# HyHuang1995/sp_orb_slam

Measured on AMD Instinct MI355X. Metric: frames/sec SuperPoint extract (752x480, 1k kpts), higher is better.
Workload: dtype f32

## Files before the change

sp_orb_slam_amd/csrc/conv_f32.hip:

```cpp
#include <type_traits>
#include <utility>

#include "spfe_kernels.h"
#include "../../include/spfe_exact_math.h"

namespace spfe {

typedef float f32x16 __attribute__((ext_vector_type(16)));

template <int KS, int TH>
struct Geo {
  static constexpr int HALO = KS / 2;
  static constexpr int ROWS = TH + 2 * HALO;
  static constexpr int COLS = 32 + 2 * HALO;
  static constexpr int ROWP = (KS == 3) ? 36 : 32;
  static constexpr int PLANE_RAW = ROWS * ROWP;
  static constexpr int PLANE = PLANE_RAW + ((2 - PLANE_RAW % 8) + 8) % 8;
};

typedef int i32x4 __attribute__((ext_vector_type(4)));
#define SPFE_OOB 0x80000000u

template <int NITER, int NWITER>
struct Pipe {
// ... 19 lines not shown
};

template <int MT, int NT, bool POOL, bool RELU, int E>
__device__ __forceinline__ void epi_store(const EpiCtx<NT> &e, const f32x16 (&acc)[MT][NT]) {
  constexpr int NEPI_ = POOL ? (MT / 2) * NT * 8 : MT * NT * 16;
  if constexpr (E >= NEPI_) {
    return;
  } else if constexpr (!POOL) {
    constexpr int j = E / (MT * 16), i = (E / 16) % MT, r = E % 16;
    constexpr int xr = (r & 3) + 8 * (r >> 2);
    float v = acc[i][j][r] + e.bias[j];
    if (RELU) v = v > 0.0f ? v : 0.0f;
    const unsigned off = (xr < e.xlim && i < e.ylim) ? e.obase[j] + i * e.rowstep + xr * e.pixstep : SPFE_OOB;
    __builtin_amdgcn_raw_buffer_store_b32(__float_as_int(v), e.rout, off, 0, 0);
  } else {
    constexpr int ip = E / (NT * 8), j = (E / 8) % NT, r = 2 * (E % 8), i0 = 2 * ip;
    constexpr int xr = (r & 3) + 8 * (r >> 2);
    float v00 = acc[i0][j][r] + e.bias[j], v01 = acc[i0][j][r + 1] + e.bias[j];
    float v10 = acc[i0 + 1][j][r] + e.bias[j], v11 = acc[i0 + 1][j][r + 1] + e.bias[j];
    if (RELU) {
      v00 = v00 > 0.0f ? v00 : 0.0f;
      v01 = v01 > 0.0f ? v01 : 0.0f;
      v10 = v10 > 0.0f ? v10 : 0.0f;
      v11 = v11 > 0.0f ? v11 : 0.0f;
    }
    const float m0 = v00 > v01 ? v00 : v01;
    const float m1 = v10 > v11 ? v10 : v11;
    const float v = m0 > m1 ? m0 : m1;
    const unsigned off = (xr < e.xlim && i0 < e.ylim) ? e.obase[j] + ip * e.rowstep + (xr >> 1) * e.pixstep : SPFE_OOB;
    __builtin_amdgcn_raw_buffer_store_b32(__float_as_int(v), e.rout, off, 0, 0);
  }
}

constexpr int F1_PROWS = 12, F1_PCOLS = 36, F1_PATCH = F1_PROWS * F1_PCOLS;

template <int NITER>
struct Fuse1a {
  float4 w[9], bias;
  float px[9];
  float4 o;
  unsigned pb[NITER];
  const float *patch;
  float *patch_next;
  const float *wsrc;
  const float *bsrc;
  __amdgpu_buffer_rsrc_t rimg;
  unsigned poff[2];
  unsigned pidx[2];
  unsigned pval[2];
  bool fill;
};
struct NoFuse {};

constexpr int F1_SUBS = 10;
template <int NITER, int IT, int SUB, int PLANE, int NWITER>
__device__ __forceinline__ void fuse_piece(Fuse1a<NITER> &z, Pipe<NITER, NWITER> &c) {
  if constexpr (SUB == 0) {
    const unsigned b = z.pb[IT] == ~0u ? 0u : z.pb[IT];
#pragma unroll
    for (int t = 0; t < 9; ++t) z.px[t] = z.patch[b + (t / 3) * F1_PCOLS + t % 3];
  } else if constexpr (SUB <= 8) {
    constexpr int j = (SUB - 1) / 2, half = (SUB - 1) % 2;
    float acc = half == 0 ? 0.0f : (j == 0 ? z.o.x : (j == 1 ? z.o.y : (j == 2 ? z.o.z : z.o.w)));
#pragma unroll
    for (int t = half * 5; t < (half == 0 ? 5 : 9); ++t) {
      const float wt = j == 0 ? z.w[t].x : (j == 1 ? z.w[t].y : (j == 2 ? z.w[t].z : z.w[t].w));
      acc = __builtin_fmaf(z.px[t], wt, acc);
    }
    if constexpr (half == 1) {
      const float bj = j == 0 ? z.bias.x : (j == 1 ? z.bias.y : (j == 2 ? z.bias.z : z.bias.w));
      acc = acc + bj;
      acc = acc > 0.0f ? acc : 0.0f;
      if (c.voff[IT] == SPFE_OOB) acc = 0.0f;
    }
    if constexpr (j == 0) z.o.x = acc;
    else if constexpr (j == 1) z.o.y = acc;
    else if constexpr (j == 2) z.o.z = acc;
    else z.o.w = acc;
  } else {
    float *d = c.nA + c.dst[IT];
    d[0] = z.o.x;
    d[PLANE] = z.o.y;
    d[2 * PLANE] = z.o.z;
    d[3 * PLANE] = z.o.w;
  }
}

template <int STEP, int NSTEP, bool FIRST, int KC, int KS, int MT, int NT, int PLANE, int ROWP, int NITER,
          int NWITER, bool POOL, bool RELU, bool FUSE, class FZ>
// ... 2 lines not shown
                                        const EpiCtx<NT> &e, FZ &fz) {
  if constexpr (STEP < NSTEP) {
    constexpr int NLDA = FUSE ? 0 : NITER;
    constexpr int NLD = NLDA + NWITER;
    constexpr int L0 = 1, W0 = NSTEP - NLD - 1;
    constexpr int NEPI = POOL ? (MT / 2) * NT * 8 : MT * NT * 16;
    constexpr int EPS = (NEPI + (NSTEP - 3)) / (NSTEP - 2);
    constexpr int cur = STEP & 1, nxt = cur ^ 1;
    static_assert(L0 + NLD <= W0, "loads and LDS writes of a stage must not overlap");
    constexpr int M = MT * NT;
#pragma unroll
    for (int m = 0; m < M; ++m) {
      if (m == 0) {
        if constexpr (STEP + 1 < NSTEP) {
          constexpr int tap = (STEP + 1) / (KC / 2), t = (STEP + 1) % (KC / 2);
          constexpr int dy = tap / KS, dx = tap % KS;
#pragma unroll
          for (int i = 0; i < MT; ++i) {
            if constexpr (KC / 2 <= 8) a[nxt][i] = c.at[t][(i + dy) * ROWP + dx];
            else a[nxt][i] = c.at[0][(2 * t) * PLANE + (i + dy) * ROWP + dx];
          }
#pragma unroll
          for (int j = 0; j < NT; ++j) bb[nxt][j] = c.bBase[j * (KS * KS * KC * 32) + (tap * KC + 2 * t) * 32];
        }
      }
      if (m == 1 % M) {
        if constexpr (STEP >= L0 && STEP - L0 < NLD) {
          constexpr int it = STEP - L0;
          if constexpr (it < NLDA) {
            const i32x4 v = __builtin_amdgcn_raw_buffer_load_b128(c.rin, c.voff[it], 0, 0);
            c.va[it] = make_float4(__int_as_float(v.x), __int_as_float(v.y), __int_as_float(v.z), __int_as_float(v.w));
          } else {
            constexpr int wi = it - NLDA;
            const i32x4 v = __builtin_amdgcn_raw_buffer_load_b128(c.rw, c.woff[wi], 0, 0);
            c.vw[wi] = make_float4(__int_as_float(v.x), __int_as_float(v.y), __int_as_float(v.z), __int_as_float(v.w));
          }
        }
      }
      if (m == 2 % M) {
        if constexpr (FIRST && STEP >= 1) {
          constexpr int e0 = (STEP - 1) * EPS;
          [&]<int... Qs>(std::integer_sequence<int, Qs...>) {
            (epi_store<MT, NT, POOL, RELU, e0 + Qs>(e, accPrev), ...);
          }(std::make_integer_sequence<int, EPS>{});
        }
      }
      if (m == 3 % M) {
        if constexpr (STEP >= W0 && STEP - W0 < NLD) {
          constexpr int it = STEP - W0;
          if constexpr (it < NLDA) {
            float *d = c.nA + c.dst[it];
            d[0] = c.va[it].x;
            d[PLANE] = c.va[it].y;
            d[2 * PLANE] = c.va[it].z;
            d[3 * PLANE] = c.va[it].w;
          } else {
            constexpr int wi = it - NLDA;
            *reinterpret_cast<float4 *>(reinterpret_cast<char *>(c.nW) + c.woff[wi]) = c.vw[wi];
          }
        }
      }
      if (m == 1 % M) {
        if constexpr (FUSE) {
          constexpr int F0 = 12;
          static_assert(L0 + NLD <= F0 && F0 + F1_SUBS * NITER <= NSTEP, "fused conv1a schedule does not fit the stage");
          if constexpr (STEP >= F0 && STEP < F0 + F1_SUBS * NITER)
            fuse_piece<NITER, (STEP - F0) / F1_SUBS, (STEP - F0) % F1_SUBS, PLANE, NWITER>(fz, c);
        }
      }
      if (m == 3 % M) {
        if constexpr (FUSE) {
          static_assert(58 < W0, "fused conv1a schedule does not fit the stage");
          if constexpr (STEP >= 2 && STEP < 11) fz.w[STEP - 2] = *reinterpret_cast<const float4 *>(fz.wsrc + (STEP - 2) * 64);
          if constexpr (STEP == 11) fz.bias = *reinterpret_cast<const float4 *>(fz.bsrc);
          if constexpr (STEP == 50) {
            if (fz.fill) {
              fz.pval[0] = __builtin_amdgcn_raw_buffer_load_b8(fz.rimg, fz.poff[0], 0, 0);
              fz.pval[1] = __builtin_amdgcn_raw_buffer_load_b8(fz.rimg, fz.poff[1], 0, 0);
            }
          }
          if constexpr (STEP == 58) {
            if (fz.fill) {
              if (fz.pidx[0] < F1_PATCH) fz.patch_next[fz.pidx[0]] = spfe_pixel_to_float((uint8_t)fz.pval[0]);
              if (fz.pidx[1] < F1_PATCH) fz.patch_next[fz.pidx[1]] = spfe_pixel_to_float((uint8_t)fz.pval[1]);
            }
          }
        }
      }
      __builtin_amdgcn_sched_barrier(0);
      {
        const int i = m / NT, j = m % NT;
        if constexpr (FIRST && STEP == 0) {
          f32x16 z;
#pragma unroll
          for (int r = 0; r < 16; ++r) z[r] = 0.0f;
          acc[i][j] = __builtin_amdgcn_mfma_f32_32x32x2f32(a[cur][i], bb[cur][j], z, 0, 0, 0);
        } else {
          acc[i][j] = __builtin_amdgcn_mfma_f32_32x32x2f32(a[cur][i], bb[cur][j], acc[i][j], 0, 0, 0);
        }
      }
      __builtin_amdgcn_sched_barrier(0);
    }
    k_steps<STEP + 1, NSTEP, FIRST, KC, KS, MT, NT, PLANE, ROWP, NITER, NWITER, POOL, RELU, FUSE, FZ>(a, bb, acc, accPrev, c, e, fz);
  }
}

template <int LAYER, int CIN, int KS, int KC, int WM, int WN, int MT, int NT, bool POOL, bool RELU>
__global__ __launch_bounds__(64 * WM * WN, 1) void conv_f32_kernel(ConvParams p) {
  constexpr int TH = WM * MT;
  using G = Geo<KS, TH>;
  constexpr int TAPS = KS * KS;
  constexpr int NCHUNK = CIN / KC;
  constexpr int PLANE = G::PLANE;
  constexpr int ROWP = G::ROWP;
  constexpr int BUF = KC * PLANE + TAPS * KC * 64;
  static_assert(WM * WN == 4 || WM * WN == 8, "4 or 8 waves per workgroup");
  constexpr int NTHR = 64 * WM * WN;
  static_assert(WN * NT == 2, "64 output channels per workgroup");
  static_assert(!POOL || MT % 2 == 0, "pooling needs row pairs per wave");
  static_assert((KC * PLANE) % 4 == 0 && BUF % 4 == 0, "weight slabs must stay 16B aligned");
  constexpr int Q = KC / 4;
  constexpr int NITEM = G::ROWS * G::COLS * Q;
  constexpr int NITER = (NITEM + NTHR - 1) / NTHR;
  constexpr int NW4 = TAPS * KC * 16;
  constexpr int NWITER = (NW4 + NTHR - 1) / NTHR;
  constexpr int NSTEP = TAPS * (KC / 2);
  constexpr int SLAB_BYTES = TAPS * KC * 64 * 4;

  constexpr bool FUSE = LAYER == 2;
  static_assert(!FUSE || (CIN == 64 && KS == 3 && KC == 16 && TH == 8), "fused conv1a is conv1b's first operand");
  using FZ = typename std::conditional<FUSE, Fuse1a<NITER>, NoFuse>::type;

  extern __shared__ __attribute__((aligned(16))) float smem[];

  const int tid = threadIdx.x;
  const int lane = tid & 63;
  const int wave = __builtin_amdgcn_readfirstlane(tid >> 6);
  const int hi = lane >> 5, l31 = lane & 31;
  const int wm = wave % WM, wn = wave / WM;
  const int H = p.H, W = p.W;

  const int total = p.nblk * p.tiles_x * p.tiles_y * p.B;
  const int first = p.item_lo, count = (p.item_hi > 0 ? p.item_hi : total) - first;
  const int xcd = blockIdx.x & 7, gi = blockIdx.x >> 3, gper = gridDim.x >> 3;
  const int lo = first + (int)((long)count * xcd / 8), hi_w = first + (int)((long)count * (xcd + 1) / 8);
  int w = lo + gi;
  if (w >= hi_w) return;

  int i_nb, i_tx, i_ty, i_b;
  {
    int t = w;
    i_nb = t % p.nblk; t /= p.nblk;
    i_tx = t % p.tiles_x; t /= p.tiles_x;
    i_ty = t % p.tiles_y; i_b = t / p.tiles_y;
  }
  int d_nb, d_tx, d_ty, d_b;
  {
    int t = gper;
    d_nb = t % p.nblk; t /= p.nblk;
    d_tx = t % p.tiles_x; t /= p.tiles_x;
    d_ty = t % p.tiles_y; d_b = t / p.tiles_y;
  }

  const unsigned in_pix_bytes = (unsigned)p.in_stride * 4u;
  const unsigned frame_in_bytes = (unsigned)H * W * in_pix_bytes;
  const int Ho = POOL ? H >> 1 : H, Wo = POOL ? W >> 1 : W;
  const unsigned out_pix_bytes = (unsigned)p.out_stride * 4u;
  const unsigned frame_out_bytes = (unsigned)Ho * Wo * out_pix_bytes;

  Pipe<NITER, NWITER> c;
  int prow[NITER], pcol[NITER];
  unsigned pqb[NITER];
#pragma unroll
  for (int it = 0; it < NITER; ++it) {
    const int i = tid + it * NTHR;
    const int qq = i % Q, pix = i / Q;
    prow[it] = i < NITEM ? pix / G::COLS - G::HALO : (1 << 20);
    pcol[it] = pix % G::COLS - G::HALO;
    pqb[it] = qq * 16;
    c.dst[it] = i < NITEM ? (qq * 4) * PLANE + (pix / G::COLS) * ROWP + pix % G::COLS
                          : (ROWP > G::COLS ? (tid % G::ROWS) * ROWP + G::COLS : G::PLANE_RAW);
  }
#pragma unroll
  for (int it = 0; it < NWITER; ++it) c.woff[it] = ((tid + it * NTHR) % NW4) * 16;

  auto aim_tile = [&](int tx, int ty) {
#pragma unroll
    for (int it = 0; it < NITER; ++it) {
      const int gy = ty * TH + prow[it], gx = tx * 32 + pcol[it];
      c.voff[it] = ((unsigned)gy < (unsigned)H && (unsigned)gx < (unsigned)W)
                       ? (unsigned)(gy * W + gx) * in_pix_bytes + pqb[it]
                       : SPFE_OOB;
    }
  };
  auto aim_stage = [&](int nb, int b, int chunk, bool valid) {
    const float *base = p.in + (size_t)b * H * W * p.in_stride + p.in_choff + chunk * KC;
    c.rin = __builtin_amdgcn_make_buffer_rsrc(const_cast<float *>(base), 0, valid ? frame_in_bytes : 0u, 0x00020000);
    const float *wb = p.wpack + ((size_t)nb * NCHUNK + chunk) * (TAPS * KC * 64);
    c.rw = __builtin_amdgcn_make_buffer_rsrc(const_cast<float *>(wb), 0, valid ? (unsigned)SLAB_BYTES : 0u, 0x00020000);
  };

  aim_tile(i_tx, i_ty);
  aim_stage(i_nb, i_b, 0, true);
  FZ fz;
  [[maybe_unused]] float *sP = smem + 2 * BUF;
  [[maybe_unused]] int pcur = 0;
  [[maybe_unused]] int php[2] = {0, 0}, pwp[2] = {0, 0};
  if constexpr (FUSE) {
    const int qq = tid % Q;
#pragma unroll
    for (int it = 0; it < NITER; ++it) {
      const int i = tid + it * 256, pix = i / Q;
      fz.pb[it] = i < NITEM ? (unsigned)((pix / G::COLS) * F1_PCOLS + pix % G::COLS) : ~0u;
    }
#pragma unroll
    for (int k = 0; k < 2; ++k) {
      const int i = tid + k * 256;
      fz.pidx[k] = i < F1_PATCH ? (unsigned)i : 0xffffu;
      php[k] = i / F1_PCOLS;
      pwp[k] = i % F1_PCOLS;
      fz.poff[k] = SPFE_OOB;
      fz.pval[k] = 0u;
    }
    fz.fill = false;
    fz.patch = sP;
    fz.patch_next = sP + F1_PATCH;
    fz.rimg = __builtin_amdgcn_make_buffer_rsrc(const_cast<uint8_t *>(p.img), 0, 0u, 0x00020000);
    fz.wsrc = p.w1a + qq * 4;
    fz.bsrc = p.b1a + qq * 4;
    {
      const uint8_t *ib = p.img + (size_t)i_b * H * W;
#pragma unroll
      for (int k = 0; k < 2; ++k) {
        const int gy = i_ty * TH - 2 + php[k], gx = i_tx * 32 - 2 + pwp[k];
        const bool in = (unsigned)gy < (unsigned)H && (unsigned)gx < (unsigned)W;
        if (fz.pidx[k] < F1_PATCH) sP[fz.pidx[k]] = in ? spfe_pixel_to_float(ib[(size_t)gy * W + gx]) : 0.0f;
      }
    }
    __syncthreads();
#pragma unroll
    for (int t = 0; t < 9; ++t) fz.w[t] = *reinterpret_cast<const float4 *>(fz.wsrc + t * 64);
    fz.bias = *reinterpret_cast<const float4 *>(fz.bsrc);
    c.nA = smem;
    [&]<int... I>(std::integer_sequence<int, I...>) {
      (fuse_piece<NITER, I / F1_SUBS, I % F1_SUBS, PLANE, NWITER>(fz, c), ...);
    }(std::make_integer_sequence<int, F1_SUBS * NITER>{});
  } else {
#pragma unroll
    for (int it = 0; it < NITER; ++it) {
      const i32x4 v = __builtin_amdgcn_raw_buffer_load_b128(c.rin, c.voff[it], 0, 0);
      c.va[it] = make_float4(__int_as_float(v.x), __int_as_float(v.y), __int_as_float(v.z), __int_as_float(v.w));
    }
  }
#pragma unroll
  for (int it = 0; it < NWITER; ++it) {
    const i32x4 v = __builtin_amdgcn_raw_buffer_load_b128(c.rw, c.woff[it], 0, 0);
    c.vw[it] = make_float4(__int_as_float(v.x), __int_as_float(v.y), __int_as_float(v.z), __int_as_float(v.w));
  }
  if constexpr (!FUSE) {
#pragma unroll
    for (int it = 0; it < NITER; ++it) {
      float *d = smem + c.dst[it];
      d[0] = c.va[it].x;
      d[PLANE] = c.va[it].y;
      d[2 * PLANE] = c.va[it].z;
      d[3 * PLANE] = c.va[it].w;
// ... 8 lines not shown
#pragma unroll
  for (int i = 0; i < MT; ++i)
#pragma unroll
    for (int j = 0; j < NT; ++j)
#pragma unroll
      for (int r = 0; r < 16; ++r) { accA[i][j][r] = 0.0f; accB[i][j][r] = 0.0f; }

  int buf = 0;
  EpiCtx<NT> epi;
  epi.rout = __builtin_amdgcn_make_buffer_rsrc(p.out, 0, 0u, 0x00020000);
#pragma unroll
  for (int j = 0; j < NT; ++j) { epi.obase[j] = SPFE_OOB; epi.bias[j] = 0.0f; }
  epi.xlim = 0; epi.ylim = 0; epi.rowstep = 0; epi.pixstep = out_pix_bytes;
  bool more = true;

  auto aim_epi = [&](EpiCtx<NT> &e, int nb, int tx, int ty, int b) {
    float *obase = p.out + (size_t)b * Ho * Wo * p.out_stride + p.out_choff;
    e.rout = __builtin_amdgcn_make_buffer_rsrc(obase, 0, frame_out_bytes, 0x00020000);
    const int y0 = ty * TH + wm * MT, x0 = tx * 32 + 4 * hi;
    e.xlim = W - x0;
    e.ylim = H - y0;
    e.rowstep = (unsigned)Wo * out_pix_bytes;
    e.pixstep = out_pix_bytes;
#pragma unroll
    for (int j = 0; j < NT; ++j) {
      const int co = nb * 64 + (wn * NT + j) * 32 + l31;
      const unsigned pix = POOL ? (unsigned)((y0 >> 1) * Wo + (x0 >> 1)) : (unsigned)(y0 * W + x0);
      e.obase[j] = co < p.cout_real ? pix * out_pix_bytes + (unsigned)co * 4u : SPFE_OOB;
      e.bias[j] = p.bias[co];
    }
  };

  EpiCtx<NT> epi_next;
  auto run_tile = [&](f32x16(&acc)[MT][NT], const f32x16(&accPrev)[MT][NT]) {
    int n_nb = i_nb + d_nb, n_tx = i_tx + d_tx, n_ty = i_ty + d_ty, n_b = i_b + d_b;
    if (n_nb >= p.nblk) { n_nb -= p.nblk; ++n_tx; }
    if (n_tx >= p.tiles_x) { n_tx -= p.tiles_x; ++n_ty; }
    if (n_ty >= p.tiles_y) { n_ty -= p.tiles_y; ++n_b; }
    const bool have_next_item = w + gper < hi_w;
    aim_epi(epi_next, i_nb, i_tx, i_ty, i_b);
#pragma unroll 1
    for (int chunk = 0; chunk < NCHUNK; ++chunk) {
      const bool last = chunk == NCHUNK - 1;
      if (!last) {
        aim_stage(i_nb, i_b, chunk + 1, true);
      } else {
        aim_tile(n_tx, n_ty);
        aim_stage(n_nb, n_b, 0, have_next_item);
      }
      if constexpr (FUSE) {
        const int produced = last ? 0 : chunk + 1;
        const int qq = tid % Q;
        fz.wsrc = p.w1a + produced * KC + qq * 4;
        fz.bsrc = p.b1a + produced * KC + qq * 4;
        fz.patch = sP + (last ? pcur ^ 1 : pcur) * F1_PATCH;
        fz.patch_next = sP + (pcur ^ 1) * F1_PATCH;
        fz.fill = chunk == NCHUNK - 2 && have_next_item;
        if (fz.fill) {
          fz.rimg = __builtin_amdgcn_make_buffer_rsrc(const_cast<uint8_t *>(p.img) + (size_t)n_b * H * W, 0,
                                                      (unsigned)(H * W), 0x00020000);
#pragma unroll
          for (int k = 0; k < 2; ++k) {
            const int gy = n_ty * TH - 2 + php[k], gx = n_tx * 32 - 2 + pwp[k];
            fz.poff[k] = ((unsigned)gy < (unsigned)H && (unsigned)gx < (unsigned)W) ? (unsigned)(gy * W + gx) : SPFE_OOB;
          }
        }
      }
      float *cA = smem + buf * BUF;
      c.nA = smem + (buf ^ 1) * BUF;
      c.nW = c.nA + KC * PLANE;
#pragma unroll
      for (int t = 0; t < (KC / 2 <= 8 ? KC / 2 : 1); ++t)
        c.at[t] = cA + (2 * t + hi) * PLANE + (wm * MT) * ROWP + l31;
      c.bBase = cA + KC * PLANE + (wn * NT) * (TAPS * KC * 32) + hi * 32 + l31;
      float a[2][MT], bb[2][NT];
#pragma unroll
      for (int i = 0; i < MT; ++i) a[0][i] = c.at[0][i * ROWP];
#pragma unroll
      for (int j = 0; j < NT; ++j) bb[0][j] = c.bBase[j * (TAPS * KC * 32)];
      if (chunk == 0)
        k_steps<0, NSTEP, true, KC, KS, MT, NT, PLANE, ROWP, NITER, NWITER, POOL, RELU, FUSE, FZ>(a, bb, acc, accPrev, c, epi, fz);
      else
        k_steps<0, NSTEP, false, KC, KS, MT, NT, PLANE, ROWP, NITER, NWITER, POOL, RELU, FUSE, FZ>(a, bb, acc, accPrev, c, epi, fz);
      __syncthreads();
      buf ^= 1;
    }
    epi = epi_next;
    if constexpr (FUSE) pcur ^= 1;
    more = have_next_item;
    w += gper;
    i_nb = n_nb; i_tx = n_tx; i_ty = n_ty; i_b = n_b;
  };

  bool lastA = true;
  while (true) {
    run_tile(accA, accB);
    lastA = true;
    if (!more) break;
    run_tile(accB, accA);
    lastA = false;
    if (!more) break;
  }
  {
    constexpr int NEPI = POOL ? (MT / 2) * NT * 8 : MT * NT * 16;
    auto flush = [&](const f32x16(&acc)[MT][NT]) {
      [&]<int... E>(std::integer_sequence<int, E...>) {
        (epi_store<MT, NT, POOL, RELU, E>(epi, acc), ...);
      }(std::make_integer_sequence<int, NEPI>{});
    };
    if (lastA) flush(accA); else flush(accB);
  }
}

template <int LAYER, int CIN, int KS, int KC, int WM, int WN, int MT, int NT, bool POOL, bool RELU>
static hipError_t launch_one(const ConvParams &p, hipStream_t s) {
  constexpr int TH = WM * MT;
  using G = Geo<KS, TH>;
  constexpr size_t lds = (2 * (size_t)(KC * G::PLANE + KS * KS * KC * 64) + (LAYER == 2 ? 2 * F1_PATCH : 0)) * sizeof(float);
  static_assert(lds <= 160 * 1024, "double buffer must fit the 160 KB LDS");
  auto k = conv_f32_kernel<LAYER, CIN, KS, KC, WM, WN, MT, NT, POOL, RELU>;
  static bool attr_done[64] = {};
  int dev = 0;
  (void)hipGetDevice(&dev);
  if (dev < 0 || dev >= 64 || !attr_done[dev]) {
    hipError_t e = hipFuncSetAttribute(reinterpret_cast<const void *>(k),
                                       hipFuncAttributeMaxDynamicSharedMemorySize, (int)lds);
    if (e != hipSuccess) return e;
    if (dev >= 0 && dev < 64) attr_done[dev] = true;
  }
  const int total = p.nblk * p.tiles_x * p.tiles_y * p.B;
  int grid = p.num_cus > 0 ? p.num_cus : 256;
  grid &= ~7;
  if (grid < 8) grid = 8;
  (void)total;
  hipLaunchKernelGGL(k, dim3(grid), dim3(64 * WM * WN), lds, s, p);
  return hipGetLastError();
}

int conv_kc(int ksize) { return ksize == 3 ? 16 : 64; }
int conv_tile_rows(int tile_mode) { return tile_mode == 1 ? 4 : (tile_mode == 2 || tile_mode == 4 ? 16 : (tile_mode == 3 ? 2 : 8)); }

hipError_t launch_conv_f32(const ConvParams &p, int cin, int ksize, bool pool, bool relu,
                           int tile_mode, int layer_tag, hipStream_t s) {
  const bool small_tile = tile_mode == 1;
  if (tile_mode == 3 && ksize == 3 && relu && !pool) {
    if (cin == 64) return launch_one<0, 64, 3, 16, 2, 2, 1, 1, false, true>(p, s);
    if (cin == 128) return launch_one<0, 128, 3, 16, 2, 2, 1, 1, false, true>(p, s);
    return hipErrorInvalidValue;
  }
  if (tile_mode == 4 && ksize == 3 && relu && pool && cin == 64 && layer_tag == 1)
    return launch_one<1, 64, 3, 16, 4, 1, 4, 2, true, true>(p, s);
  if (tile_mode == 2 && ksize == 3 && relu) {
    if (layer_tag == 1 && cin == 64 && pool) return launch_one<1, 64, 3, 16, 8, 1, 2, 2, true, true>(p, s);
    if (cin == 64 && pool) return launch_one<0, 64, 3, 16, 8, 1, 2, 2, true, true>(p, s);
    if (cin == 64 && !pool) return launch_one<0, 64, 3, 16, 8, 1, 2, 2, false, true>(p, s);
    if (cin == 128 && pool) return launch_one<0, 128, 3, 16, 8, 1, 2, 2, true, true>(p, s);
    if (cin == 128 && !pool) return launch_one<0, 128, 3, 16, 8, 1, 2, 2, false, true>(p, s);
    return hipErrorInvalidValue;
  }
  if (layer_tag == 1 && cin == 64 && ksize == 3 && pool && relu && !small_tile)
    return launch_one<1, 64, 3, 16, 4, 1, 2, 2, true, true>(p, s);
  if (layer_tag == 2 && cin == 64 && ksize == 3 && pool && relu && !small_tile && p.img && p.w1a && p.b1a)
    return launch_one<2, 64, 3, 16, 4, 1, 2, 2, true, true>(p, s);
#define SPFE_CONV(CIN_, KS_, KC_, WM_, WN_, MT_, NT_, POOL_, RELU_)                       \
  if (cin == CIN_ && ksize == KS_ && pool == POOL_ && relu == RELU_ &&                    \
      small_tile == (WM_ * MT_ == 4))                                                     \
    return launch_one<0, CIN_, KS_, KC_, WM_, WN_, MT_, NT_, POOL_, RELU_>(p, s);
  SPFE_CONV(64, 3, 16, 4, 1, 2, 2, true, true)
  SPFE_CONV(64, 3, 16, 4, 1, 2, 2, false, true)
  SPFE_CONV(128, 3, 16, 4, 1, 2, 2, true, true)
  SPFE_CONV(128, 3, 16, 4, 1, 2, 2, false, true)
  SPFE_CONV(64, 3, 16, 2, 2, 2, 1, true, true)
  SPFE_CONV(64, 3, 16, 2, 2, 2, 1, false, true)
  SPFE_CONV(128, 3, 16, 2, 2, 2, 1, true, true)
  SPFE_CONV(128, 3, 16, 2, 2, 2, 1, false, true)
  SPFE_CONV(256, 1, 64, 2, 2, 2, 1, false, false)
#undef SPFE_CONV
  return hipErrorInvalidValue;
}

__global__ __launch_bounds__(256) void conv1a_kernel(const uint8_t *__restrict__ img,
                                                     const float *__restrict__ w9x64,
                                                     const float *__restrict__ b64,
                                                     float *__restrict__ out, int B, int H, int W,
// ... 91 lines not shown
```

sp_orb_slam_amd/csrc/spfe_schedule.hip:

```cpp
#include "spfe_host.h"

namespace spfe_host {

hipError_t wait_if_pending(hipStream_t s, hipEvent_t ev) {
  hipStreamCaptureStatus cs = hipStreamCaptureStatusNone;
  if (hipStreamIsCapturing(s, &cs) == hipSuccess && cs == hipStreamCaptureStatusNone) {
    const hipError_t q = hipEventQuery(ev);
    if (q == hipSuccess) return hipSuccess;
    if (q != hipErrorNotReady) (void)hipGetLastError();
  }
  return hipStreamWaitEvent(s, ev, 0);
}

#define STAGE_MARK(i) \
  do { if (h->timing && (h->timing_all || (i) == 1 || (i) == 2)) HIP_TRY(hipEventRecord(h->ev[i], s)); } while (0)

}
namespace spfe {
__global__ void copy_records_kernel(uint4 *dst, const uint4 *src, size_t n16) {
  for (size_t i = (size_t)blockIdx.x * blockDim.x + threadIdx.x; i < n16; i += (size_t)gridDim.x * blockDim.x) dst[i] = src[i];
  __threadfence_system();
}

__global__ void queue_probe_spin_kernel(long long ticks, long long *stamp) {
// ... 56 lines not shown
    const int q2 = q1 == 0 ? streams_share_a_queue(c, h->side, h->probe_stamp) : q1;
    if (q1 < 0 || q2 < 0) h->split_probe = -1;
    if (q1 == 0 && q2 == 0) {
      h->conv2 = c;
      h->conv2_ok = true;
      h->split_probe = 1;
      break;
    }
  }
  return SPFE_OK;
}

int settle_join(spfe_handle h, hipStream_t s) {
  if (h->join_pending) {
    HIP_TRY(wait_if_pending(s, h->ev_join));
    h->join_pending = false;
  }
  return SPFE_OK;
}

int enqueue(spfe_handle h, const uint8_t *d_images, int n, uint8_t *d_records, hipStream_t s) {
  const int H = h->H, W = h->W;
  if (h->open_n) return fail(SPFE_EINVAL, "a call begun by spfe_extract_begin is open: spfe_extract_finish first");
  if (h->timing) h->ev = h->evpool.data() + (size_t)(h->calls % spfe_handle_s::EVSETS) * (NSTAGE + 1);
  h->calls++;
  h->host_sync_n = 0;
  STAGE_MARK(0);
  if (h->bf16) { const int rcj = settle_join(h, s); if (rcj) return rcj; }
  if (h->d_tile_ctr && !h->tile_ctr_clean) {
    hipLaunchKernelGGL(spfe::zero_tile_counters_kernel, dim3(1), dim3(256), 0, s, h->d_tile_ctr, 8 * 64);
    HIP_TRY(hipGetLastError());
  }
  h->tile_ctr_clean = false;
  const bool fused = !h->bf16 && (h->fuse1a || (h->fuse1a_env < 0 && n == 1 && !((h->cfg.flags & SPFE_FLAG_ASYNC_COV) || h->pipe_mode) &&
                                                !(h->timing && h->timing_all)));
  const int grid_ws0 = std::max(16, (h->num_cus > 0 ? h->num_cus : 256) & ~15);
  const int ws_min = ((h->cfg.flags & SPFE_FLAG_ASYNC_COV) || h->pipe_mode) ? h->ws_min_items : h->ws_min_items_sync;
  const bool ws_layer0 = h->bf16 && h->d_wws[0] && W >= 32 &&
                         (long)((W + 31) / 32) * ((H + 7) / 8) * n >= (long)ws_min * grid_ws0;
  const bool fused16 = ws_layer0 && h->fuse1a_bf16;
  h->act0_missing = fused || fused16;
  bool early_waits = false;
  {
    if (h->early_waits && h->split_last && h->pbtail && n >= 2 && ((h->cfg.flags & SPFE_FLAG_ASYNC_COV) || h->pipe_mode) && !(h->timing && h->timing_all)) {
      const int rcw = tail_waits(h, d_records, s);
      if (rcw) return rcw;
      early_waits = true;
    }
  }
  if (h->bf16 && !fused16) HIP_TRY(spfe::launch_conv1a_bf16(d_images, h->d_w1a_tab, h->d_b1a, h->act[0], n, H, W, s));
  else if (!h->bf16 && !fused) HIP_TRY(spfe::launch_conv1a(d_images, h->d_w1a, h->d_b1a, h->act[0], n, H, W, s));
  { const int rcj = settle_join(h, s); if (rcj) return rcj; }
  STAGE_MARK(1);
  const int n_all = n;
  hipStream_t const s_all = s;
  const bool sparse = h->sparse_db && h->d_db_list && !(h->sparse_db_sync_only && ((h->cfg.flags & SPFE_FLAG_ASYNC_COV) || h->pipe_mode));
  const bool sparse_da = sparse && h->sparse_da && (h->sparse_da_mode >= 2 || !((h->cfg.flags & SPFE_FLAG_ASYNC_COV) || h->pipe_mode));
  h->sparse_da_call = sparse_da;
  const int par_db = (int)(h->ticket & 1);
  h->feat_cur = sparse_da && par_db ? h->act7_alt : h->act[7];
  bool tail_per_half = false;
  auto run_layer = [&](int i, int f0 = 0, int nfr = -1, hipStream_t s_use = nullptr) -> int {
    const ConvLayer &L = h->layers[i];
    hipStream_t s = s_use ? s_use : s_all;
    const int n = nfr < 0 ? n_all : nfr;
    if (i == 9 && h->desc_recorded) HIP_TRY(wait_if_pending(s, h->ev_desc));
    if (!sparse_da && i == 7 && h->dbs_recorded[par_db ^ 1]) HIP_TRY(wait_if_pending(s, h->ev_dbs[par_db ^ 1]));
    if (sparse_da && i == 6 && h->dbs_recorded[par_db]) HIP_TRY(wait_if_pending(s, h->ev_dbs[par_db]));
// ... 99 lines not shown
      const long tx = (L.W + 31) / 32;
      const long nblk_eff = i == 7 && sparse_da ? L.nblk / 2 : L.nblk;
      const long items_big = tx * ((L.H + 7) / 8) * nblk_eff * n, items_small = tx * ((L.H + 3) / 4) * nblk_eff * n;
      const long g = h->num_cus > 0 ? h->num_cus : 256;
      const double cost_big = (double)((items_big + g - 1) / g) * 2.0 * 0.93;
      const double cost_small = (double)((items_small + g - 1) / g);
      small_tile = cost_small < cost_big;
      if (!L.pool && L.relu && !(i == 0 && fused) && h->tile2_auto) {
        const long items_tiny = tx * ((L.H + 1) / 2) * nblk_eff * n;
        const double cost_tiny = (double)((items_tiny + g - 1) / g) * 0.56;
        tiny_tile = cost_tiny < (cost_small < cost_big ? cost_small : cost_big);
      }
    }
    bool pool_split = false;
    if (L.ks == 3 && L.pool && L.relu && i > 0 && i < 7 && h->d_unpooled && h->pool_split != 0 && n_all == 1 &&
         !(L.H & 1) && !(L.W & 1) &&
        (size_t)n * L.H * L.W * L.out_stride <= (size_t)std::min(h->B, 2) * (H / 2) * (W / 2) * 64) {
      const long tx = (L.W + 31) / 32, g = h->num_cus > 0 ? h->num_cus : 256;
      const long items_big = tx * ((L.H + 7) / 8) * L.nblk * n, items_small = tx * ((L.H + 3) / 4) * L.nblk * n;
      const long items_tiny = tx * ((L.H + 1) / 2) * L.nblk * n;
      const double cost_big = (double)((items_big + g - 1) / g) * 2.0 * 0.93, cost_small = (double)((items_small + g - 1) / g);
      const double cost_tiny = (double)((items_tiny + g - 1) / g) * 0.56 + 0.12;
      pool_split = h->pool_split > 0 || cost_tiny < (cost_small < cost_big ? cost_small : cost_big) - 0.02;
    }
    if (pool_split) {
      spfe::ConvParams q = p;
      q.out = h->d_unpooled; q.out_stride = L.out_stride; q.out_choff = 0;
      q.tiles_x = (L.W + 31) / 32; q.tiles_y = (L.H + 1) / 2; q.nblk = L.nblk; q.num_cus = h->num_cus;
      HIP_TRY(spfe::launch_conv_f32(q, L.cin, L.ks, false, true, 3, 0, s));
      HIP_TRY(spfe::launch_pool2x2_f32(h->d_unpooled, p.out, n, L.H, L.W, L.out_stride, s));
      STAGE_MARK(2 + i);
      return SPFE_OK;
    }
    if (i == 0 && fused) small_tile = false;
    int tile_mode = small_tile ? 1 : 0;
    long split16_rows = -1;
    if (i == 0 && !fused && L.pool && h->tile16x4 && (tile_mode == 0 || h->tile16x4 == 2)) {
      const long g = h->num_cus > 0 ? h->num_cus : 256;
      const long tx = (L.W + 31) / 32, ty8 = (L.H + 7) / 8, ty16 = (L.H + 15) / 16;
      const long r8 = (tx * ty8 * n + g - 1) / g, r16 = (tx * ty16 * n + g - 1) / g;
      const double c8 = (double)r8, c16 = 2.0 * r16 * 0.975;
      double best = c8 < c16 ? c8 : c16;
      if (c16 < c8 || h->tile16x4 == 2) tile_mode = 4;
      if (h->tile16x4 == 1 && r8 >= 8)
        for (long k = ty16 * n - 1; k > 0 && k >= ty16 * n - 4 * ty16; --k) {
          const long f = k / ty16, r = k % ty16;
          const long rows8 = (ty8 - std::min(2 * r, ty8)) + (n - f - 1) * ty8;
          const double c = 2.0 * ((tx * k + g - 1) / g) * 0.975 + (double)((tx * rows8 + g - 1) / g) + 0.3;
          if (c < best - 0.2) { best = c; split16_rows = k; }
        }
    }
    if (tiny_tile && tile_mode != 2 && tile_mode != 4) tile_mode = 3;
    if (L.ks == 3 && !L.pool && L.relu && ((h->tile2_mask >> i) & 1)) tile_mode = 3;
    const int th = spfe::conv_tile_rows(tile_mode);
    if (i == 0) { h->conv1b_tile_rows = th; h->conv1b_split_rows = (int)split16_rows; }
    p.tiles_x = (L.W + 31) / 32; p.tiles_y = (L.H + th - 1) / th; p.nblk = L.nblk;
    if (i == 7 && sparse_da) p.nblk = L.nblk / 2;
    p.num_cus = h->num_cus;
    if (split16_rows > 0) {
      const int ty8 = (L.H + 7) / 8, ty16 = (L.H + 15) / 16;
      const long f = split16_rows / ty16, r = split16_rows % ty16;
      spfe::ConvParams p16 = p;
      p16.tiles_y = ty16;
      p16.item_lo = 0; p16.item_hi = (int)(p.tiles_x * split16_rows);
      HIP_TRY(spfe::launch_conv_f32(p16, L.cin, L.ks, L.pool, L.relu, 4, 1, s));
      const bool kernel_bracket = h->timing && !h->timing_all;
      if (kernel_bracket) HIP_TRY(hipEventRecord(h->ev[2], s));
      p.tiles_y = ty8;
      p.item_lo = (int)((f * ty8 + std::min<long>(2 * r, ty8)) * p.tiles_x);
      p.item_hi = p.tiles_x * ty8 * n;
      h->conv1b_tile_rows = 16;
      HIP_TRY(spfe::launch_conv_f32(p, L.cin, L.ks, L.pool, L.relu, 0, 1, s));
      if (!kernel_bracket) STAGE_MARK(2 + i);
      return SPFE_OK;
    }
    HIP_TRY(spfe::launch_conv_f32(p, L.cin, L.ks, L.pool, L.relu, tile_mode, i == 0 ? (fused ? 2 : 1) : 0, s));
    STAGE_MARK(2 + i);
    return SPFE_OK;
  };
  const bool defer_db = !sparse && !(h->timing && h->timing_all) && h->defer_db && !((h->cfg.flags & SPFE_FLAG_ASYNC_COV) || h->pipe_mode);
  const int nlayers = sparse ? 9 : 10;
  bool split = (h->split_mode >= 0 ? h->split_mode >= 1 : (!h->bf16 || h->C < 10000)) && !(!h->bf16 && h->f32_heads) && n >= 2 && !(h->timing && h->timing_all) && !defer_db;
  if (split) {
    const int rcp = pick_conv2(h, s);
    if (rcp) return rcp;
    split = h->conv2_ok;
  }
  h->split_last = split;
  if (split) {
    tail_per_half = h->pbtail && h->tail_per_half;
    if (tail_per_half && !early_waits) {
      const int rcw = tail_waits(h, d_records, s);
      if (rcw) return rcw;
    }
    int rc = run_layer(0);
    if (rc) return rc;
    HIP_TRY(hipEventRecord(h->ev_fork, s));
    HIP_TRY(hipStreamWaitEvent(h->conv2, h->ev_fork, 0));
    const int parts = 2;
    for (int q = 0; q < parts; q += 2)
      for (int i = 1; i < nlayers; ++i)
        for (int r = q; r < std::min(q + 2, parts); ++r) {
          const int f0 = (int)((long)n * r / parts), f1 = (int)((long)n * (r + 1) / parts);
          if ((rc = run_layer(i, f0, f1 - f0, (r & 1) ? h->conv2 : s))) return rc;
        }
// ... 242 lines not shown
```

Before: 2148.

## Add lean fused conv1a path for 16-row conv1b tiles and auto-enable fusion

Adds a new 'lean' variant of the fused conv1a-into-conv1b kernel for the 16x4 tile mode. It uses a packed per-channel tap table in LDS, a uint8 image patch, and a re-spread sub-step schedule across MFMA slots. The host schedule now plans the conv1b tile mode before deciding on fusion, and enables fusion whenever the 16-row or split plan is chosen. This is meant to remove the separate conv1a launch and its activation round trip through memory for batched or larger inputs. The cost is more LDS use, extra VALU work interleaved with the MFMAs, and added complexity in the schedule.

```diff
diff --git a/sp_orb_slam_amd/csrc/conv_f32.hip b/sp_orb_slam_amd/csrc/conv_f32.hip
--- a/sp_orb_slam_amd/csrc/conv_f32.hip
+++ b/sp_orb_slam_amd/csrc/conv_f32.hip
@@ -75,10 +75,14 @@
   }
 }
 
-constexpr int F1_PROWS = 12, F1_PCOLS = 36, F1_PATCH = F1_PROWS * F1_PCOLS;
-
-template <int NITER>
+constexpr int F1_PCOLS = 36;
+constexpr int f1_patch(int th) { return (th + 4) * F1_PCOLS; }
+constexpr int f1_fill(int th) { return (f1_patch(th) + 255) / 256; }
+
+template <int NITER, int TH>
 struct Fuse1a {
+  static constexpr bool LEAN = false;
+  static constexpr int PATCH = f1_patch(TH), NPF = f1_fill(TH);
   float4 w[9], bias;
   float px[9];
   float4 o;
@@ -88,16 +92,82 @@
   const float *wsrc;
   const float *bsrc;
   __amdgpu_buffer_rsrc_t rimg;
-  unsigned poff[2];
-  unsigned pidx[2];
-  unsigned pval[2];
+  unsigned poff[NPF];
+  unsigned pidx[NPF];
+  unsigned pval[NPF];
   bool fill;
 };
-struct NoFuse {};
+struct NoFuse { static constexpr bool LEAN = false; };
+
+constexpr int F1L_TAPW = 12;
+constexpr int F1L_TAPS = 64 * F1L_TAPW;
+template <int NITER, int TH>
+struct Fuse1aL {
+  static constexpr bool LEAN = true;
+  static constexpr int PATCH = f1_patch(TH), NPF = f1_fill(TH);
+  float px[9];
+  float o[4];
+  float4 wa, wb;
+  float2 wc;
+  unsigned oob;
+  unsigned pix0;
+  int qoff;
+  const uint8_t *patch;
+  uint8_t *patch_next;
+  const float *taps;
+  __amdgpu_buffer_rsrc_t rimg;
+  unsigned poff[NPF];
+  unsigned pval[NPF];
+  bool fill;
+};
+
+constexpr int F1L_SUBS = 12;
+template <int NITER, int IT, int SUB, int PLANE, int NWITER, int TH>
+__device__ __forceinline__ void fuse_piece_lean(Fuse1aL<NITER, TH> &z, Pipe<NITER, NWITER> &c) {
+  if constexpr (SUB == 0) {
+    const uint8_t *s = z.patch + (c.dst[IT] - z.qoff);
+#pragma unroll
+    for (int t = 0; t < 9; ++t) z.px[t] = __uint_as_float((unsigned)s[(t / 3) * F1_PCOLS + t % 3]);
+  } else if constexpr (SUB <= 2) {
+#pragma unroll
+    for (int t = (SUB == 1 ? 0 : 5); t < (SUB == 1 ? 5 : 9); ++t) z.px[t] = spfe_pixel_to_float((uint8_t)__float_as_uint(z.px[t]));
+    if constexpr (SUB == 2) z.wa = *reinterpret_cast<const float4 *>(z.taps);
+  } else if constexpr (SUB <= 10) {
+    constexpr int j = (SUB - 3) / 2, half = (SUB - 3) % 2;
+    if constexpr (half == 0) {
+      float acc = 0.0f;
+      acc = __builtin_fmaf(z.px[0], z.wa.x, acc);
+      acc = __builtin_fmaf(z.px[1], z.wa.y, acc);
+      acc = __builtin_fmaf(z.px[2], z.wa.z, acc);
+      acc = __builtin_fmaf(z.px[3], z.wa.w, acc);
+      z.o[j] = acc;
+      z.wb = *reinterpret_cast<const float4 *>(z.taps + j * F1L_TAPW + 4);
+      z.wc = *reinterpret_cast<const float2 *>(z.taps + j * F1L_TAPW + 8);
+    } else {
+      float acc = z.o[j];
+      acc = __builtin_fmaf(z.px[4], z.wb.x, acc);
+      acc = __builtin_fmaf(z.px[5], z.wb.y, acc);
+      acc = __builtin_fmaf(z.px[6], z.wb.z, acc);
+      acc = __builtin_fmaf(z.px[7], z.wb.w, acc);
+      acc = __builtin_fmaf(z.px[8], z.wc.x, acc);
+      acc = acc + z.wc.y;
+      acc = acc > 0.0f ? acc : 0.0f;
+      if (z.oob & (1u << IT)) acc = 0.0f;
+      z.o[j] = acc;
+      if constexpr (j < 3) z.wa = *reinterpret_cast<const float4 *>(z.taps + (j + 1) * F1L_TAPW);
+    }
+  } else {
+    float *d = c.nA + c.dst[IT];
+    d[0] = z.o[0];
+    d[PLANE] = z.o[1];
+    d[2 * PLANE] = z.o[2];
+    d[3 * PLANE] = z.o[3];
+  }
+}
 
 constexpr int F1_SUBS = 10;
-template <int NITER, int IT, int SUB, int PLANE, int NWITER>
-__device__ __forceinline__ void fuse_piece(Fuse1a<NITER> &z, Pipe<NITER, NWITER> &c) {
+template <int NITER, int IT, int SUB, int PLANE, int NWITER, int TH>
+__device__ __forceinline__ void fuse_piece(Fuse1a<NITER, TH> &z, Pipe<NITER, NWITER> &c) {
   if constexpr (SUB == 0) {
     const unsigned b = z.pb[IT] == ~0u ? 0u : z.pb[IT];
 #pragma unroll
@@ -166,7 +236,8 @@
             c.va[it] = make_float4(__int_as_float(v.x), __int_as_float(v.y), __int_as_float(v.z), __int_as_float(v.w));
           } else {
             constexpr int wi = it - NLDA;
-            const i32x4 v = __builtin_amdgcn_raw_buffer_load_b128(c.rw, c.woff[wi], 0, 0);
+            const i32x4 v = FZ::LEAN ? __builtin_amdgcn_raw_buffer_load_b128(c.rw, c.woff[0], wi * 4096, 0)
+                                     : __builtin_amdgcn_raw_buffer_load_b128(c.rw, c.woff[wi], 0, 0);
             c.vw[wi] = make_float4(__int_as_float(v.x), __int_as_float(v.y), __int_as_float(v.z), __int_as_float(v.w));
           }
         }
@@ -190,33 +261,59 @@
             d[3 * PLANE] = c.va[it].w;
           } else {
             constexpr int wi = it - NLDA;
-            *reinterpret_cast<float4 *>(reinterpret_cast<char *>(c.nW) + c.woff[wi]) = c.vw[wi];
-          }
-        }
-      }
-      if (m == 1 % M) {
-        if constexpr (FUSE) {
+            *reinterpret_cast<float4 *>(reinterpret_cast<char *>(c.nW) + (FZ::LEAN ? c.woff[0] + wi * 4096 : c.woff[wi])) = c.vw[wi];
+          }
+        }
+      }
+      if constexpr (FUSE && !FZ::LEAN) {
+        if (m == 1 % M) {
           constexpr int F0 = 12;
           static_assert(L0 + NLD <= F0 && F0 + F1_SUBS * NITER <= NSTEP, "fused conv1a schedule does not fit the stage");
           if constexpr (STEP >= F0 && STEP < F0 + F1_SUBS * NITER)
             fuse_piece<NITER, (STEP - F0) / F1_SUBS, (STEP - F0) % F1_SUBS, PLANE, NWITER>(fz, c);
         }
-      }
-      if (m == 3 % M) {
-        if constexpr (FUSE) {
+        if (m == 3 % M) {
           static_assert(58 < W0, "fused conv1a schedule does not fit the stage");
           if constexpr (STEP >= 2 && STEP < 11) fz.w[STEP - 2] = *reinterpret_cast<const float4 *>(fz.wsrc + (STEP - 2) * 64);
           if constexpr (STEP == 11) fz.bias = *reinterpret_cast<const float4 *>(fz.bsrc);
           if constexpr (STEP == 50) {
             if (fz.fill) {
-              fz.pval[0] = __builtin_amdgcn_raw_buffer_load_b8(fz.rimg, fz.poff[0], 0, 0);
-              fz.pval[1] = __builtin_amdgcn_raw_buffer_load_b8(fz.rimg, fz.poff[1], 0, 0);
+#pragma unroll
+              for (int k = 0; k < FZ::NPF; ++k) fz.pval[k] = __builtin_amdgcn_raw_buffer_load_b8(fz.rimg, fz.poff[k], 0, 0);
             }
           }
           if constexpr (STEP == 58) {
             if (fz.fill) {
-              if (fz.pidx[0] < F1_PATCH) fz.patch_next[fz.pidx[0]] = spfe_pixel_to_float((uint8_t)fz.pval[0]);
-              if (fz.pidx[1] < F1_PATCH) fz.patch_next[fz.pidx[1]] = spfe_pixel_to_float((uint8_t)fz.pval[1]);
+#pragma unroll
+              for (int k = 0; k < FZ::NPF; ++k)
+                if (fz.pidx[k] < FZ::PATCH) fz.patch_next[fz.pidx[k]] = spfe_pixel_to_float((uint8_t)fz.pval[k]);
+            }
+          }
+        }
+      }
+      if constexpr (FUSE && FZ::LEAN) {
+        constexpr int F0 = 2, s0 = (STEP - F0) * 2, NSUB = F1L_SUBS * NITER;
+        static_assert(M == 8 && F0 * 2 + NSUB <= NSTEP * 2, "fused conv1a schedule does not fit the stage");
+        if constexpr (STEP >= F0) {
+          if (m == 4) {
+            if constexpr (s0 < NSUB) fuse_piece_lean<NITER, s0 / F1L_SUBS, s0 % F1L_SUBS, PLANE, NWITER>(fz, c);
+          }
+          if (m == 6) {
+            if constexpr (s0 + 1 < NSUB) fuse_piece_lean<NITER, (s0 + 1) / F1L_SUBS, (s0 + 1) % F1L_SUBS, PLANE, NWITER>(fz, c);
+          }
+        }
+        if (m == 5) {
+          if constexpr (STEP == 0) {
+            if (fz.fill) {
+#pragma unroll
+              for (int k = 0; k < FZ::NPF; ++k) fz.pval[k] = __builtin_amdgcn_raw_buffer_load_b8(fz.rimg, fz.poff[k], 0, 0);
+            }
+          }
+          if constexpr (STEP == 8) {
+            if (fz.fill) {
+#pragma unroll
+              for (int k = 0; k < FZ::NPF; ++k)
+                if (fz.pix0 + k * 256 < (unsigned)FZ::PATCH) fz.patch_next[fz.pix0 + k * 256] = (uint8_t)fz.pval[k];
             }
           }
         }
@@ -262,8 +359,12 @@
   constexpr int SLAB_BYTES = TAPS * KC * 64 * 4;
 
   constexpr bool FUSE = LAYER == 2;
-  static_assert(!FUSE || (CIN == 64 && KS == 3 && KC == 16 && TH == 8), "fused conv1a is conv1b's first operand");
-  using FZ = typename std::conditional<FUSE, Fuse1a<NITER>, NoFuse>::type;
+  static_assert(!FUSE || (CIN == 64 && KS == 3 && KC == 16 && (TH == 8 || TH == 16) && NTHR == 256), "fused conv1a is conv1b's first operand");
+  static_assert(!FUSE || F1L_TAPS % NTHR == 0, "the tap table is filled in whole passes");
+  constexpr bool LEAN = FUSE && TH == 16;
+  static_assert(!LEAN || (NW4 % NTHR == 0 && NTHR * 16 == 4096), "weight piece it = piece 0 + it * 4096 bytes");
+  using FZ = typename std::conditional<FUSE, typename std::conditional<LEAN, Fuse1aL<NITER, TH>, Fuse1a<NITER, TH>>::type, NoFuse>::type;
+  constexpr int F1_PATCH = f1_patch(TH), F1_NPF = f1_fill(TH);
 
   extern __shared__ __attribute__((aligned(16))) float smem[];
 
@@ -314,17 +415,30 @@
     pqb[it] = qq * 16;
     c.dst[it] = i < NITEM ? (qq * 4) * PLANE + (pix / G::COLS) * ROWP + pix % G::COLS
                           : (ROWP > G::COLS ? (tid % G::ROWS) * ROWP + G::COLS : G::PLANE_RAW);
+    if constexpr (LEAN) if (i >= NITEM) c.dst[it] = (qq * 4) * PLANE + (tid % (G::ROWS - 1)) * ROWP + G::COLS;
   }
 #pragma unroll
   for (int it = 0; it < NWITER; ++it) c.woff[it] = ((tid + it * NTHR) % NW4) * 16;
 
+  [[maybe_unused]] unsigned oob_next = 0;
   auto aim_tile = [&](int tx, int ty) {
-#pragma unroll
-    for (int it = 0; it < NITER; ++it) {
-      const int gy = ty * TH + prow[it], gx = tx * 32 + pcol[it];
-      c.voff[it] = ((unsigned)gy < (unsigned)H && (unsigned)gx < (unsigned)W)
-                       ? (unsigned)(gy * W + gx) * in_pix_bytes + pqb[it]
-                       : SPFE_OOB;
+    if constexpr (LEAN) {
+      const int qoff = ((tid % Q) * 4) * PLANE;
+      oob_next = 0;
+#pragma unroll
+      for (int it = 0; it < NITER; ++it) {
+        const int r = (c.dst[it] - qoff) / ROWP, col = (c.dst[it] - qoff) % ROWP;
+        const int gy = ty * TH - G::HALO + r, gx = tx * 32 - G::HALO + col;
+        if (!((unsigned)gy < (unsigned)H && (unsigned)gx < (unsigned)W)) oob_next |= 1u << it;
+      }
+    } else {
+#pragma unroll
+      for (int it = 0; it < NITER; ++it) {
+        const int gy = ty * TH + prow[it], gx = tx * 32 + pcol[it];
+        c.voff[it] = ((unsigned)gy < (unsigned)H && (unsigned)gx < (unsigned)W)
+                         ? (unsigned)(gy * W + gx) * in_pix_bytes + pqb[it]
+                         : SPFE_OOB;
+      }
     }
   };
   auto aim_stage = [&](int nb, int b, int chunk, bool valid) {
@@ -339,17 +453,53 @@
   FZ fz;
   [[maybe_unused]] float *sP = smem + 2 * BUF;
   [[maybe_unused]] int pcur = 0;
-  [[maybe_unused]] int php[2] = {0, 0}, pwp[2] = {0, 0};
-  if constexpr (FUSE) {
+  [[maybe_unused]] int php[F1_NPF] = {}, pwp[F1_NPF] = {};
+  [[maybe_unused]] float *sT = smem + 2 * BUF;
+  [[maybe_unused]] uint8_t *sPb = reinterpret_cast<uint8_t *>(smem + 2 * BUF + F1L_TAPS);
+  [[maybe_unused]] auto aim_patch = [&](int tx, int ty, unsigned (&off)[F1_NPF]) __attribute__((always_inline)) {
+#pragma unroll
+    for (int k = 0; k < F1_NPF; ++k) {
+      const int i = tid + k * NTHR;
+      const int gy = ty * TH - 2 + i / F1_PCOLS, gx = tx * 32 - 2 + i % F1_PCOLS;
+      off[k] = ((unsigned)gy < (unsigned)H && (unsigned)gx < (unsigned)W) ? (unsigned)(gy * W + gx) : SPFE_OOB;
+    }
+  };
+  if constexpr (LEAN) {
     const int qq = tid % Q;
+    fz.oob = oob_next;
+    fz.qoff = (qq * 4) * PLANE;
+    fz.pix0 = (unsigned)tid;
+    fz.fill = false;
+    fz.patch = sPb;
+    fz.patch_next = sPb + F1_PATCH;
+    fz.taps = sT + (qq * 4) * F1L_TAPW;
+#pragma unroll
+    for (int k = 0; k < F1L_TAPS / NTHR; ++k) {
+      const int i = tid + k * NTHR, ch = i / F1L_TAPW, e = i % F1L_TAPW;
+      sT[i] = e < 9 ? p.w1a[e * 64 + ch] : (e == 9 ? p.b1a[ch] : 0.0f);
+    }
+    fz.rimg = __builtin_amdgcn_make_buffer_rsrc(const_cast<uint8_t *>(p.img) + (size_t)i_b * H * W, 0, (unsigned)(H * W), 0x00020000);
+    aim_patch(i_tx, i_ty, fz.poff);
+#pragma unroll
+    for (int k = 0; k < F1_NPF; ++k) {
+      fz.pval[k] = __builtin_amdgcn_raw_buffer_load_b8(fz.rimg, fz.poff[k], 0, 0);
+      if (fz.pix0 + k * 256 < (unsigned)F1_PATCH) sPb[fz.pix0 + k * 256] = (uint8_t)fz.pval[k];
+    }
+    __syncthreads();
+    c.nA = smem;
+    [&]<int... I>(std::integer_sequence<int, I...>) {
+      (fuse_piece_lean<NITER, I / F1L_SUBS, I % F1L_SUBS, PLANE, NWITER>(fz, c), ...);
+    }(std::make_integer_sequence<int, F1L_SUBS * NITER>{});
+  } else if constexpr (FUSE) {
+    const int qq = tid % Q;
 #pragma unroll
     for (int it = 0; it < NITER; ++it) {
-      const int i = tid + it * 256, pix = i / Q;
+      const int i = tid + it * NTHR, pix = i / Q;
       fz.pb[it] = i < NITEM ? (unsigned)((pix / G::COLS) * F1_PCOLS + pix % G::COLS) : ~0u;
     }
 #pragma unroll
-    for (int k = 0; k < 2; ++k) {
-      const int i = tid + k * 256;
+    for (int k = 0; k < F1_NPF; ++k) {
+      const int i = tid + k * NTHR;
       fz.pidx[k] = i < F1_PATCH ? (unsigned)i : 0xffffu;
       php[k] = i / F1_PCOLS;
       pwp[k] = i % F1_PCOLS;
@@ -365,7 +515,7 @@
     {
       const uint8_t *ib = p.img + (size_t)i_b * H * W;
 #pragma unroll
-      for (int k = 0; k < 2; ++k) {
+      for (int k = 0; k < F1_NPF; ++k) {
         const int gy = i_ty * TH - 2 + php[k], gx = i_tx * 32 - 2 + pwp[k];
         const bool in = (unsigned)gy < (unsigned)H && (unsigned)gx < (unsigned)W;
         if (fz.pidx[k] < F1_PATCH) sP[fz.pidx[k]] = in ? spfe_pixel_to_float(ib[(size_t)gy * W + gx]) : 0.0f;
@@ -440,7 +590,7 @@
   };
 
   EpiCtx<NT> epi_next;
-  auto run_tile = [&](f32x16(&acc)[MT][NT], const f32x16(&accPrev)[MT][NT]) {
+  auto run_tile = [&](f32x16(&acc)[MT][NT], const f32x16(&accPrev)[MT][NT]) __attribute__((always_inline)) {
     int n_nb = i_nb + d_nb, n_tx = i_tx + d_tx, n_ty = i_ty + d_ty, n_b = i_b + d_b;
     if (n_nb >= p.nblk) { n_nb -= p.nblk; ++n_tx; }
     if (n_tx >= p.tiles_x) { n_tx -= p.tiles_x; ++n_ty; }
@@ -456,7 +606,19 @@
         aim_tile(n_tx, n_ty);
         aim_stage(n_nb, n_b, 0, have_next_item);
       }
-      if constexpr (FUSE) {
+      if constexpr (LEAN) {
+        const int produced = last ? 0 : chunk + 1;
+        if (last) fz.oob = oob_next;
+        fz.taps = sT + (produced * KC + (tid % Q) * 4) * F1L_TAPW;
+        fz.patch = sPb + (last ? pcur ^ 1 : pcur) * F1_PATCH;
+        fz.patch_next = sPb + (pcur ^ 1) * F1_PATCH;
+        fz.fill = chunk == NCHUNK - 2 && have_next_item;
+        if (fz.fill) {
+          fz.rimg = __builtin_amdgcn_make_buffer_rsrc(const_cast<uint8_t *>(p.img) + (size_t)n_b * H * W, 0,
+                                                      (unsigned)(H * W), 0x00020000);
+          aim_patch(n_tx, n_ty, fz.poff);
+        }
+      } else if constexpr (FUSE) {
         const int produced = last ? 0 : chunk + 1;
         const int qq = tid % Q;
         fz.wsrc = p.w1a + produced * KC + qq * 4;
@@ -468,7 +630,7 @@
           fz.rimg = __builtin_amdgcn_make_buffer_rsrc(const_cast<uint8_t *>(p.img) + (size_t)n_b * H * W, 0,
                                                       (unsigned)(H * W), 0x00020000);
 #pragma unroll
-          for (int k = 0; k < 2; ++k) {
+          for (int k = 0; k < F1_NPF; ++k) {
             const int gy = n_ty * TH - 2 + php[k], gx = n_tx * 32 - 2 + pwp[k];
             fz.poff[k] = ((unsigned)gy < (unsigned)H && (unsigned)gx < (unsigned)W) ? (unsigned)(gy * W + gx) : SPFE_OOB;
           }
@@ -524,7 +686,8 @@
 static hipError_t launch_one(const ConvParams &p, hipStream_t s) {
   constexpr int TH = WM * MT;
   using G = Geo<KS, TH>;
-  constexpr size_t lds = (2 * (size_t)(KC * G::PLANE + KS * KS * KC * 64) + (LAYER == 2 ? 2 * F1_PATCH : 0)) * sizeof(float);
+  constexpr size_t lds = 2 * (size_t)(KC * G::PLANE + KS * KS * KC * 64) * sizeof(float) +
+                         (LAYER != 2 ? 0 : TH == 16 ? F1L_TAPS * sizeof(float) + 2 * f1_patch(TH) : 2 * f1_patch(TH) * sizeof(float));
   static_assert(lds <= 160 * 1024, "double buffer must fit the 160 KB LDS");
   auto k = conv_f32_kernel<LAYER, CIN, KS, KC, WM, WN, MT, NT, POOL, RELU>;
   static bool attr_done[64] = {};
@@ -558,6 +721,8 @@
   }
   if (tile_mode == 4 && ksize == 3 && relu && pool && cin == 64 && layer_tag == 1)
     return launch_one<1, 64, 3, 16, 4, 1, 4, 2, true, true>(p, s);
+  if (tile_mode == 4 && ksize == 3 && relu && pool && cin == 64 && layer_tag == 2 && p.img && p.w1a && p.b1a)
+    return launch_one<2, 64, 3, 16, 4, 1, 4, 2, true, true>(p, s);
   if (tile_mode == 2 && ksize == 3 && relu) {
     if (layer_tag == 1 && cin == 64 && pool) return launch_one<1, 64, 3, 16, 8, 1, 2, 2, true, true>(p, s);
     if (cin == 64 && pool) return launch_one<0, 64, 3, 16, 8, 1, 2, 2, true, true>(p, s);
diff --git a/sp_orb_slam_amd/csrc/spfe_schedule.hip b/sp_orb_slam_amd/csrc/spfe_schedule.hip
--- a/sp_orb_slam_amd/csrc/spfe_schedule.hip
+++ b/sp_orb_slam_amd/csrc/spfe_schedule.hip
@@ -112,8 +112,43 @@
     HIP_TRY(hipGetLastError());
   }
   h->tile_ctr_clean = false;
-  const bool fused = !h->bf16 && (h->fuse1a || (h->fuse1a_env < 0 && n == 1 && !((h->cfg.flags & SPFE_FLAG_ASYNC_COV) || h->pipe_mode) &&
-                                                !(h->timing && h->timing_all)));
+  struct Conv1bPlan { int tile_mode; long split16_rows; };
+  auto plan_conv1b = [&](bool no_small) -> Conv1bPlan {
+    const ConvLayer &L = h->layers[0];
+    const long g = h->num_cus > 0 ? h->num_cus : 256;
+    const long tx = (L.W + 31) / 32, ty8 = (L.H + 7) / 8, ty16 = (L.H + 15) / 16;
+    bool small_tile = L.small_tile;
+    if (L.ks == 3 && h->small_maxh < 0) {
+      const long items_big = tx * ty8 * L.nblk * n, items_small = tx * ((L.H + 3) / 4) * L.nblk * n;
+      small_tile = (double)((items_small + g - 1) / g) < (double)((items_big + g - 1) / g) * 2.0 * 0.93;
+    }
+    if (no_small) small_tile = false;
+    Conv1bPlan pl{small_tile ? 1 : 0, -1};
+    if (L.pool && h->tile16x4 && (pl.tile_mode == 0 || h->tile16x4 == 2)) {
+      const long r8 = (tx * ty8 * n + g - 1) / g, r16 = (tx * ty16 * n + g - 1) / g;
+      const double c8 = (double)r8, c16 = 2.0 * r16 * 0.975;
+      double best = c8 < c16 ? c8 : c16;
+      if (c16 < c8 || h->tile16x4 == 2) pl.tile_mode = 4;
+      if (h->tile16x4 == 1 && r8 >= 8)
+        for (long k = ty16 * n - 1; k > 0 && k >= ty16 * n - 4 * ty16; --k) {
+          const long f = k / ty16, r = k % ty16;
+          const long rows8 = (ty8 - std::min(2 * r, ty8)) + (n - f - 1) * ty8;
+          const double c = 2.0 * ((tx * k + g - 1) / g) * 0.975 + (double)((tx * rows8 + g - 1) / g) + 0.3;
+          if (c < best - 0.2) { best = c; pl.split16_rows = k; }
+        }
+    }
+    return pl;
+  };
+  Conv1bPlan plan1b{0, -1};
+  bool fused = false;
+  if (!h->bf16) {
+    plan1b = plan_conv1b(h->fuse1a);
+    fused = h->fuse1a;
+    if (h->fuse1a_env < 0 && !(h->timing && h->timing_all)) {
+      if (plan1b.tile_mode == 4 || plan1b.split16_rows > 0) fused = true;
+      else if (n == 1 && !((h->cfg.flags & SPFE_FLAG_ASYNC_COV) || h->pipe_mode)) { fused = true; plan1b = plan_conv1b(true); }
+    }
+  }
   const int grid_ws0 = std::max(16, (h->num_cus > 0 ? h->num_cus : 256) & ~15);
   const int ws_min = ((h->cfg.flags & SPFE_FLAG_ASYNC_COV) || h->pipe_mode) ? h->ws_min_items : h->ws_min_items_sync;
   const bool ws_layer0 = h->bf16 && h->d_wws[0] && W >= 32 &&
@@ -279,24 +314,9 @@
       STAGE_MARK(2 + i);
       return SPFE_OK;
     }
-    if (i == 0 && fused) small_tile = false;
     int tile_mode = small_tile ? 1 : 0;
     long split16_rows = -1;
-    if (i == 0 && !fused && L.pool && h->tile16x4 && (tile_mode == 0 || h->tile16x4 == 2)) {
-      const long g = h->num_cus > 0 ? h->num_cus : 256;
-      const long tx = (L.W + 31) / 32, ty8 = (L.H + 7) / 8, ty16 = (L.H + 15) / 16;
-      const long r8 = (tx * ty8 * n + g - 1) / g, r16 = (tx * ty16 * n + g - 1) / g;
-      const double c8 = (double)r8, c16 = 2.0 * r16 * 0.975;
-      double best = c8 < c16 ? c8 : c16;
-      if (c16 < c8 || h->tile16x4 == 2) tile_mode = 4;
-      if (h->tile16x4 == 1 && r8 >= 8)
-        for (long k = ty16 * n - 1; k > 0 && k >= ty16 * n - 4 * ty16; --k) {
-          const long f = k / ty16, r = k % ty16;
-          const long rows8 = (ty8 - std::min(2 * r, ty8)) + (n - f - 1) * ty8;
-          const double c = 2.0 * ((tx * k + g - 1) / g) * 0.975 + (double)((tx * rows8 + g - 1) / g) + 0.3;
-          if (c < best - 0.2) { best = c; split16_rows = k; }
-        }
-    }
+    if (i == 0) { tile_mode = plan1b.tile_mode; split16_rows = plan1b.split16_rows; }
     if (tiny_tile && tile_mode != 2 && tile_mode != 4) tile_mode = 3;
     if (L.ks == 3 && !L.pool && L.relu && ((h->tile2_mask >> i) & 1)) tile_mode = 3;
     const int th = spfe::conv_tile_rows(tile_mode);
@@ -310,14 +330,14 @@
       spfe::ConvParams p16 = p;
       p16.tiles_y = ty16;
       p16.item_lo = 0; p16.item_hi = (int)(p.tiles_x * split16_rows);
-      HIP_TRY(spfe::launch_conv_f32(p16, L.cin, L.ks, L.pool, L.relu, 4, 1, s));
+      HIP_TRY(spfe::launch_conv_f32(p16, L.cin, L.ks, L.pool, L.relu, 4, fused ? 2 : 1, s));
       const bool kernel_bracket = h->timing && !h->timing_all;
       if (kernel_bracket) HIP_TRY(hipEventRecord(h->ev[2], s));
       p.tiles_y = ty8;
       p.item_lo = (int)((f * ty8 + std::min<long>(2 * r, ty8)) * p.tiles_x);
       p.item_hi = p.tiles_x * ty8 * n;
       h->conv1b_tile_rows = 16;
-      HIP_TRY(spfe::launch_conv_f32(p, L.cin, L.ks, L.pool, L.relu, 0, 1, s));
+      HIP_TRY(spfe::launch_conv_f32(p, L.cin, L.ks, L.pool, L.relu, 0, fused ? 2 : 1, s));
       if (!kernel_bracket) STAGE_MARK(2 + i);
       return SPFE_OK;
     }
```

Result: slower. 2042 (-4.9%).
